# nmdp-bioinformatics/py-graph-imputation

Measured on AMD Instinct MI355X. Metric: imputed subjects/sec (whole node), 5-locus CAU graph, higher is better.
Workload: dtype f64; 1 GPU; BASELINE configs[1]: CAU 5-locus graph, 10k synthetic fully-typed subjects; 10000 subjects per step and GPU, seed=rank; graph_nodes=35411, populations=1

## Files before the change

include/grim_hip.h:

```cpp
#ifndef GRIM_HIP_H
#define GRIM_HIP_H

#include <stddef.h>
#include <stdint.h>

#ifdef __cplusplus
extern "C" {
#endif

#define GRIM_MAXL 5
#define GRIM_ABITS 12
#define GRIM_KEY_GRAPH_ORDER 60
#define GRIM_MAXPH 16
#define GRIM_MAXPOP 64
#define GRIM_TOPCAP 128
#define GRIM_MAXLADDER 64
#define GRIM_MAXROWS 8

typedef struct grim_ctx grim_ctx;
typedef struct grim_graph grim_graph;
typedef struct grim_batch grim_batch;

grim_ctx *grim_create(int device_id);
void grim_destroy(grim_ctx *ctx);
// ... 194 lines not shown

typedef struct {
  uint64_t lines, subjects, chunks, reruns;
  uint64_t unsupported;
  double wall_s;
  double tokenize_cpu_s, format_cpu_s, write_cpu_s;
  double device_s;
  double kernel_ms[7];
  uint64_t counters[4];
  uint64_t text_bytes[7];
  uint64_t bytes_h2d, bytes_d2h;
} grim_stream_stats;

grim_stream *grim_stream_open(grim_ctx *ctx, const grim_graph *g, const grim_dict *dict, const grim_params *prm,
                              const grim_prior_spec *priors, const char *const *pop_names, uint32_t n_pops,
                              const grim_stream_opts *opts);
int grim_stream_write(grim_stream *s, const char *text, uint64_t len);
int grim_stream_write_borrowed(grim_stream *s, const char *text, uint64_t len);
int grim_stream_write_text(grim_stream *s, const char *text, uint64_t len);
int grim_stream_write_file(grim_stream *s, const char *path);
int grim_stream_segment(grim_stream *s, uint64_t next_line_offset);
uint32_t grim_stream_n_segments(const grim_stream *s);
int grim_stream_segment_end(const grim_stream *s, uint32_t k, uint64_t out[7]);
int grim_stream_segment_wait(grim_stream *s, uint32_t k, uint64_t sizes[7]);
int grim_stream_segment_place(grim_stream *s, uint32_t k, const uint64_t base[6]);
int64_t grim_chunk_offsets(const char *path, uint32_t chunk_lines, uint64_t **out);
void grim_free(void *p);
uint32_t grim_default_threads(void);
int grim_stream_finish(grim_stream *s);
const char *grim_stream_error(const grim_stream *s);
const char *grim_stream_text(grim_stream *s, int which, uint64_t *len);
int grim_stream_get_stats(const grim_stream *s, grim_stream_stats *out);
int grim_stream_devtok_lines(const grim_stream *s, uint64_t *offered, uint64_t *handed_back);
uint32_t grim_tokname_hash(const char *name, uint32_t len);
uint64_t grim_stream_n_unsupported(const grim_stream *s);
int grim_stream_unsupported(const grim_stream *s, uint64_t k, uint64_t *line, uint32_t *reason, const char **id, uint32_t *id_len);
typedef struct {
  uint64_t first_line;
  uint32_t n_lines;
  const uint8_t *kinds;
  const grim_subject_result *res;
  const grim_row *rows;
  void *chunk;
} grim_stream_records;
int grim_stream_next_records(grim_stream *s, grim_stream_records *out);
int grim_stream_release_records(grim_stream *s, grim_stream_records *rec);
void grim_stream_free(grim_stream *s);

typedef struct grim_em grim_em;
typedef struct {
  uint64_t key;
  double w;
  uint32_t batch;
  uint32_t subject, row;
  uint16_t pop, side;
} grim_em_spill_rec;
grim_em *grim_em_create(grim_ctx *ctx, const uint32_t n_alleles[GRIM_MAXL], uint32_t n_pops, uint64_t first_capacity);
int grim_em_accumulate(grim_em *em, grim_batch *b);
int grim_em_accumulate_records(grim_em *em, const grim_subject_result *res, uint32_t n_subjects, const grim_row *rows,
                               uint64_t n_rows);
uint64_t grim_em_entries(const grim_em *em);
int grim_em_export(grim_em *em, uint64_t *keys, uint32_t *pops, double *counts);
uint64_t grim_em_spill_count(const grim_em *em);
int grim_em_spill(grim_em *em, uint64_t first, uint64_t n, grim_em_spill_rec *out);
int grim_em_stats(const grim_em *em, uint64_t out[4]);
uint64_t grim_em_last_unsupported(const grim_em *em);
// ... 83 lines not shown
```

py-graph-imputation_amd/csrc/grim_engine.hip:

```cpp
#include <hip/hip_runtime.h>
#include <hip/hip_ext.h>
#include <stdio.h>
#include <stdlib.h>
#include <string.h>
#include <algorithm>
#include <atomic>
#include <mutex>
#include <string>
#include <vector>

#include "grim_plan_a.h"
#include "grim_plan_b.h"
#include "grim_small.h"
#include "grim_medium.h"
#include "grim_mid.h"
#include "grim_tables.h"
#include "grim_tokdev.h"
#include "grim_em.h"
#include "grim_refresh.h"
#include "grim_marginal.h"
#include "grim_match.h"
#include "grim_search.h"
#include "grim_engine_internal.h"
#include "grim_host_internal.h"
#include "grim_sdma.h"

__global__ __launch_bounds__(GRIM_WG, GRIM_WG_PER_CU) void grim_plan_a_kernel(DevArgs A) {
  __shared__ WgShared sh;
  __shared__ WaveTop wt[GRIM_NWAVE];
  const int tid = threadIdx.x;
  const int P = A.g.P;
  Slot S = make_slot(A, blockIdx.x);
  const uint32_t n_bail = A.bail_list ? A.queue[GRIM_Q_BAIL] : 0, n_bail_heavy = A.bail_list ? A.queue[GRIM_Q_BAIL_HEAVY] : 0;
  const uint32_t n_mid = A.mid_list ? A.queue[GRIM_Q_MID] : 0;
  if (tid < GRIM_NWAVE * 4) ((unsigned long long *)sh.wctr)[tid] = 0;
  wg_arena(sh, wt);
  __syncthreads();
  for (;;) {
    if (tid == 0) sh.bc[3] = atomicAdd(A.queue + GRIM_Q_GENERAL, 1u);
    __syncthreads();
    const uint32_t w = sh.bc[3];
    if (A.mid_list ? w >= n_mid : w >= A.n_work + n_bail + n_bail_heavy) break;
    uint32_t si;
    if (A.mid_list)
      si = A.mid_list[w];
    else if (w < n_bail_heavy)
      si = A.bail_list[A.n_medium - 1u - w];
    else if (w - n_bail_heavy < A.n_work)
      si = A.order[w - n_bail_heavy];
    else
// ... 1189 lines not shown
  if (g2 == 0) g2 = 1;
  static int bucket_per_cu = 0;
  if (bucket_per_cu == 0) {
    int nb = 0;
    if (hipOccupancyMaxActiveBlocksPerMultiprocessor(&nb, grim_tables_bucket_kernel, 64, 0) != hipSuccess || nb <= 0) {
      (void)hipGetLastError();
      nb = 8;
    }
    bucket_per_cu = nb > 32 ? 32 : nb;
  }
  const uint32_t g3 = (uint32_t)c->n_cu * (uint32_t)bucket_per_cu;
  uint32_t g4 = (uint32_t)c->n_cu * (160u * 1024u / (uint32_t)sizeof(SplitWave)), g5 = (uint32_t)c->n_cu * 16u;
  if (g4 > cand) g4 = cand;
  if (g5 > cand) g5 = cand;
  if (g4 == 0) g4 = 1;
  if (g5 == 0) g5 = 1;
  (void)hipMemsetAsync(c->wctr, 0, 4 * GRIM_WCTR_WORDS, c->stream);
  launch_span(b, PH_TABLES, true, false, grim_tables_wave_kernel, dim3(g1), dim3(64), A);
  launch(b, PH_NONE, grim_tables_split_wave_kernel, dim3(g4), dim3(64), A);
  launch(b, PH_NONE, grim_tables_split_kernel, dim3(g2), dim3(GRIM_WG), A);
  launch(b, PH_NONE, grim_tables_bucket_kernel, dim3(g3), dim3(64), A);
  launch(b, PH_NONE, grim_tables_merge_wave_kernel, dim3(g5), dim3(64), A);
  launch_span(b, PH_TABLES, false, true, grim_tables_merge_kernel, dim3(g2), dim3(GRIM_WG), A);
}

static void enqueue_half_wave(grim_batch *b, bool timed, const DevArgs &Ak, const SmallRec *recs, const uint32_t *order, uint32_t n, uint32_t stage) {
  const uint32_t per_block = GRIM_WG / 32;
  launch(b, timed ? PH_HALF_WAVE : PH_NONE, grim_plan_a_small_kernel, dim3((n + per_block - 1) / per_block), dim3(GRIM_WG), Ak, recs, n, stage,
         b->small_stride);
  launch(b, timed ? PH_COMPACT : PH_NONE, grim_small_compact_kernel, dim3((n + 63) / 64), dim3(64), b->a, order, order ? nullptr : recs, n, stage,
         b->small_stride);
}

static int enqueue_stage1(grim_batch *b) {
  grim_ctx *c = b->ctx;
  DevArgs &A = b->a;
  const uint32_t stage0 = (uint32_t)b->row_limit - (b->n_small + b->n_dev_lines) * b->small_stride;
  if (b->n_small) enqueue_half_wave(b, b->n_dev_lines == 0, A, b->d_small, b->d_os, b->n_small, stage0);
  if (b->n_dev_lines) {
    DevTok T;
    T.text = b->d_text;
    T.lines = b->d_lines;
    T.lo = b->dev_lo;
    T.hi = b->dev_hi;
    T.dict = b->dict->d;
    T.dsmall = b->d_dsmall;
    T.subj = const_cast<grim_subject *>(A.subj);
    T.tok = const_cast<uint16_t *>(A.tok);
    T.tok_base = (uint32_t)(b->plan.tok_cap ? b->plan.tok_cap : 1);
    T.graph_loci = A.g.n_loci;
    const dim3 tgrid((b->n_dev_lines + (GRIM_WG / 64) * TOK_LINES_PER_WAVE - 1) / ((GRIM_WG / 64) * TOK_LINES_PER_WAVE));
    launch(b, PH_TOKENIZER, grim_tokenize_kernel, tgrid, dim3(GRIM_WG), A, T);
    DevArgs A2 = A;
    A2.small_ctr = A.small_ctr + 2 * b->n_host_small_waves;
    enqueue_half_wave(b, true, A2, b->d_dsmall, nullptr, b->n_dev_lines, stage0 + b->n_small * b->small_stride);
  }
  if (b->n_medium) {
    static const int waves_per_cu = env_int("GRIM_MEDIUM_WAVES", GRIM_MEDIUM_WAVES_PER_CU);
    uint32_t grid = (uint32_t)c->n_cu * (uint32_t)(waves_per_cu > 0 ? waves_per_cu : GRIM_MEDIUM_WAVES_PER_CU);
    if (grid > b->n_medium) grid = b->n_medium;
    launch(b, PH_ONE_WAVE, grim_plan_a_medium_kernel, dim3(grid), dim3(64), A, b->d_om, b->n_medium, A.bail_list);
  }
  if (A.mid_list && b->n_general + b->n_medium) {
    const uint32_t want = b->n_general + b->n_medium;
    uint32_t grid = (uint32_t)c->n_cu * GRIM_MID_WG_PER_CU;
    if (grid > want) grid = want;
    launch(b, PH_MID, grim_plan_a_mid_kernel, dim3(grid), dim3(GRIM_WG), A);
  }
  if (b->n_general + b->n_medium) {
    uint32_t want = b->n_general + b->n_medium;
    launch(b, PH_GENERAL, grim_plan_a_kernel, dim3(b->n_slots < want ? b->n_slots : want), dim3(GRIM_WG), A);
  }
  launch(b, PH_NONE, grim_finish_kernel, dim3(1), dim3(GRIM_WG), A.counters, b->hstate, 0u, 0);
  return hipGetLastError() == hipSuccess ? 0 : -1;
}

extern "C" int grim_batch_set_timing(grim_batch *b, int on) {
  if (!b) return -1;
  b->timing = on != 0;
  memset(b->acc_ms, 0, sizeof(b->acc_ms));
  b->n_timed = 0;
  return 0;
}

int engine_batch_upload_done(grim_batch *b) {
  if (!b || !b->up_pending) return 1;
  use_device(b->ctx->device);
  if (hipEventQuery(b->ev_up) == hipSuccess) return 1;
  (void)hipGetLastError();
  return 0;
}

int engine_batch_enqueue(grim_batch *b) {
  if (!b) return -1;
  grim_ctx *c = b->ctx;
  use_device(c->device);
  if (((uint64_t)b->n_small + b->n_dev_lines) * b->small_stride > b->row_limit) {
    b->rows_used = 0;
    set_err(c, "grim_batch_run: output row pool smaller than the half-wave kernel's fixed region");
    return -2;
  }
  memset(b->ms, 0, sizeof(b->ms));
  b->launched = 0;
  std::lock_guard<std::mutex> lk(c->run_mu);
  if (bind_scratch(b) != 0) return -1;
  if (b->up_pending) {
    b->up_pending = false;
    if (hipEventQuery(b->ev_up) != hipSuccess) {
      (void)hipGetLastError();
      HIPCHK(hipStreamWaitEvent(c->stream, b->ev_up, 0), c, -1);
    }
  }
  if (b->timing) {
    if (enqueue_stage1(b) != 0) {
      set_err(c, "grim_batch_run: kernel launch failed");
      return -1;
    }
  } else {
    if (b->graph_state == 0) {
      b->graph_state = -1;
      static const int use_graph = env_int("GRIM_GRAPH", 0);
      if (use_graph && hipStreamBeginCapture(c->stream, hipStreamCaptureModeThreadLocal) == hipSuccess) {
        int rc = enqueue_stage1(b);
        hipGraph_t gr = nullptr;
        hipError_t e = hipStreamEndCapture(c->stream, &gr);
        if (rc == 0 && e == hipSuccess && gr && hipGraphInstantiate(&b->gexec, gr, nullptr, nullptr, 0) == hipSuccess)
          b->graph_state = 1;
        if (gr) hipGraphDestroy(gr);
        (void)hipGetLastError();
      }
// ... 1463 lines not shown
```

py-graph-imputation_amd/csrc/grim_engine_internal.h:

```cpp
#pragma once
#include <stdint.h>

#include "../../include/grim_hip.h"
#include "grim_layout.h"
#include "grim_tok.h"

struct EnginePlan {
  uint32_t n_subj;
  uint64_t tok_cap;
  uint64_t text_cap;
};

struct EngineHost {
  grim_subject *subj;
  uint16_t *tok;
  SmallRec *small;
  uint32_t *order_s, *order_m, *order_g;
  grim_subject_result *res;
  grim_row *rows;
  LineRec *lines;
  uint8_t *text;
};

struct EngineLoad {
  uint32_t n_subj;
  uint32_t n_small, n_medium, n_general;
  uint64_t tok_used;
  uint32_t n_priors;
  const double *priors;
  uint32_t dev_lo, dev_hi;
  uint64_t text_bytes;
};

grim_batch *engine_batch_create(grim_ctx *ctx, const grim_graph *g, const grim_params *p, uint64_t row_limit, const EnginePlan *plan);
int engine_batch_plan(grim_batch *b, const EnginePlan *plan);
const EngineHost *engine_batch_host(grim_batch *b);
uint32_t engine_small_stride(const grim_params *p);
uint64_t engine_rows_per_subject(const grim_params *p, uint32_t n_pops);
int engine_batch_load(grim_batch *b, const EngineLoad *ld);
int engine_batch_fetch(grim_batch *b, uint32_t res_lo, uint32_t res_hi, grim_row *rows_dst);
uint64_t engine_bytes_moved(const grim_batch *b, int dir);
void engine_set_error(grim_ctx *ctx, const char *msg);
void engine_batch_recycle(grim_batch *b);
int engine_batch_fetch_issue(grim_batch *b);
int engine_batch_fetch_wait(grim_batch *b);
int engine_batch_upload_done(grim_batch *b);
int engine_batch_enqueue(grim_batch *b);
int engine_batch_wait(grim_batch *b);
struct DictSnap;
typedef struct grim_devdict grim_devdict;
grim_devdict *engine_devdict_create(grim_ctx *ctx, const DictSnap *snap);
void engine_devdict_free(grim_devdict *d);
void engine_batch_set_dict(grim_batch *b, const grim_devdict *d);
uint32_t engine_batch_irregular(const grim_batch *b);
uint32_t engine_graph_order_bad(const grim_graph *g);
uint64_t engine_batch_pool_want(const grim_batch *b);
void engine_batch_hint_pool(grim_batch *b, uint64_t records);
int engine_batch_grow_pool(grim_batch *b, uint64_t max_records);
int engine_batch_grow_rows(grim_batch *b, uint64_t max_rows);
uint64_t engine_batch_row_limit(const grim_batch *b);
void engine_batch_hint_rows(grim_batch *b, uint64_t rows);
```

py-graph-imputation_amd/csrc/grim_small.h:

```cpp
#pragma once
#include "grim_pair.h"


__device__ __forceinline__ double half_shfl_d(double v, int src_in_half) {
  return __shfl(v, (threadIdx.x & 32) | src_in_half);
}
__device__ __forceinline__ uint32_t half_shfl_u(uint32_t v, int src_in_half) {
  return __shfl(v, (threadIdx.x & 32) | src_in_half);
}

template <int CTRL>
__device__ __forceinline__ double dpp_d(double v) {
  const long long b = __double_as_longlong(v);
  const int lo = __builtin_amdgcn_update_dpp(0, (int)(uint32_t)b, CTRL, 0xF, 0xF, false);
  const int hi = __builtin_amdgcn_update_dpp(0, (int)(uint32_t)((unsigned long long)b >> 32), CTRL, 0xF, 0xF, false);
  return __longlong_as_double((long long)(((unsigned long long)(uint32_t)hi << 32) | (uint32_t)lo));
}
__device__ __forceinline__ double row16_max(double v) {
  double o;
  o = dpp_d<0x121>(v); v = o > v ? o : v;
  o = dpp_d<0x122>(v); v = o > v ? o : v;
  o = dpp_d<0x124>(v); v = o > v ? o : v;
  o = dpp_d<0x128>(v); v = o > v ? o : v;
  return v;
}

__global__ __launch_bounds__(GRIM_WG) void grim_plan_a_small_kernel(DevArgs A, const SmallRec *recs, uint32_t n,
                                                                   uint32_t row_base, uint32_t row_stride) {
  const DevGraph &g = A.g;
  const int hl = threadIdx.x & 31;
  const uint32_t w = blockIdx.x * (GRIM_WG / 32) + (threadIdx.x >> 5);
  bool live = w < n;
  const int n_ladder = A.prm.n_ladder;
  double lad[8];
#pragma unroll
  for (int i = 0; i < 8; ++i) lad[i] = A.prm.ladder[i];
  bool hit = false;
  uint64_t mykey = 0;
  double f = 0.0;
  uint32_t same = 0, si = 0;
  double w_prior = 0.0;
  if (live) {
    const uint4 *rp = (const uint4 *)(recs + w);
    const uint4 r0 = rp[0], r1 = rp[1];
    const uint32_t words[8] = {r0.x, r0.y, r0.z, r0.w, r1.x, r1.y, r1.z, r1.w};
    same = (words[6] >> 8) & 0xFFu;
    si = words[7];
    live = si != GRIM_NONE;
    w_prior = live ? A.priors[(uint64_t)(words[6] >> 16)] : 0.0;
#pragma unroll
    for (int l = 0; l < GRIM_MAXL; ++l) {
      const uint32_t tw = words[l];
      const uint32_t t = ((hl >> l) & 1) ? (tw >> 16) : (tw & 0xFFFFu);
      const uint32_t slot = (l < 4 ? (words[5] >> (8 * l)) : words[6]) & 0xFFu;
      mykey |= (uint64_t)(t + 1u) << (GRIM_ABITS * slot);
    }
    uint32_t h = fht_hash(mykey) & g.fht_mask;
    for (; live;) {
      const FullEnt e = g.fht[h];
      if (e.key == mykey) { hit = true; f = e.f0; break; }
      if (e.key == 0) break;
      h = (h + 1) & g.fht_mask;
    }
  }
  const bool hit2 = half_shfl_u(hit ? 1u : 0u, hl ^ 31) != 0;
  const double f2 = half_shfl_d(f, hl ^ 31);
  const uint64_t key2 = ((uint64_t)half_shfl_u((uint32_t)(mykey >> 32), hl ^ 31) << 32) | half_shfl_u((uint32_t)mykey, hl ^ 31);
  const uint32_t het4 = 15u & ~same;
  bool kept = hl < 16 && ((uint32_t)hl & ~het4 & 15u) == 0 && (!((same >> 4) & 1u) || ((uint32_t)hl ^ het4) >= (uint32_t)hl);
  const bool pair_ok = live && kept && f > 0.0 && f2 > 0.0;
  const bool same_hap = mykey == key2;
  PairRef pr;
  pr.p1 = f; pr.p2 = f2; pr.m2 = f2;
  pr.e1 = same_hap ? 0u : 1u; pr.e2 = 0u;
  const bool hi_half = (threadIdx.x & 32) != 0;
  double eps = 0.0;
// ... 16 lines not shown
    for (int idx = 0; idx < 8; ++idx)
      if (idx < n_ladder && (need_lo || need_hi)) step(lad[idx]);
    for (int idx = 8; idx < n_ladder && (need_lo || need_hi); ++idx) step(A.prm.ladder[idx]);
    eps = hi_half ? eps_hi : eps_lo;
    found = hi_half ? got_hi : got_lo;
  }
  double prob = acc ? pair_prob(pr, w_prior) : 0.0;
  double mx = row16_max(prob);
  if (found && eps > 0.0) {
    eps = mx / 100000.0;
    acc = pair_ok && pair_accept(eps, pr, w_prior);
    prob = acc ? pair_prob(pr, w_prior) : 0.0;
    mx = row16_max(prob);
  }
  const uint64_t bal = __ballot(acc);
  const uint32_t accmask = (uint32_t)(hi_half ? (bal >> 32) : bal) & 0xFFFFu;
  const uint32_t nU = __popc(accmask);
  double total = 0.0;
  bool first = true;
  uint32_t rank = 0;
  for (uint32_t um = ((uint32_t)bal | (uint32_t)(bal >> 32)) & 0xFFFFu; um; um &= um - 1) {
    const int i = __builtin_ctz(um);
    const double p_lo = lane_get(prob, i), p_hi = lane_get(prob, 32 + i);
    const double pi = hi_half ? p_hi : p_lo;
    if ((accmask >> i) & 1u) {
      total = first ? pi : total + pi;
      first = false;
      if (pi > prob || (pi == prob && i < hl)) ++rank;
    }
  }
  {
    const uint64_t need = __ballot(live && kept), needp = __ballot(live && kept && hit),
                   needq = __ballot(live && kept && hit2);
    if ((threadIdx.x & 63) == 0) {
      const uint32_t gw = blockIdx.x * (GRIM_WG / 64) + (threadIdx.x >> 6);
      *(uint2 *)(A.small_ctr + 2 * gw) = make_uint2(2u * (uint32_t)__popcll(need), (uint32_t)(__popcll(needp) + __popcll(needq)));
    }
  }
  if (!live) return;
  const uint32_t off = row_base + w * row_stride;
  const bool ok = nU > 0;
  const int first_lane = ok ? (__ffs(accmask) - 1) : 0;
  const uint32_t n_pm = (ok && A.prm.out_haps) ? (nU < A.prm.n_results ? nU : A.prm.n_results) : 0;
  const uint64_t ka = ((uint64_t)half_shfl_u((uint32_t)(mykey >> 32), first_lane) << 32) | half_shfl_u((uint32_t)mykey, first_lane);
  const uint64_t kb = ((uint64_t)half_shfl_u((uint32_t)(key2 >> 32), first_lane) << 32) | half_shfl_u((uint32_t)key2, first_lane);
  {
    const int f = hl - 16;
    const bool phase = hl < 16;
    const bool wr = ok && (phase ? (acc && rank < n_pm) : f == 0);
    if (wr) {
      grim_row r;
      r.a = phase ? mykey : ka;
      r.b = phase ? key2 : kb;
      r.prob = phase ? prob : total;
      r.popa = 0;
      r.popb = 0;
      A.rows[off + (phase ? GRIM_SMALL_ROWS_FIXED + rank : (uint32_t)f)] = r;
    }
  }
  if (hl >= 19 && hl < 26) {
    const int j = hl - 19;
    const uint8_t status = ok ? GRIM_ST_OK : (A.prm.planb ? GRIM_ST_UNSUPPORTED : GRIM_ST_MISS);
    const uint32_t head = (uint32_t)status | ((uint32_t)'a' << 8) | ((!ok && A.prm.planb) ? (2u << 16) : 0u);
    const uint32_t n_um = (ok && A.prm.out_muug && A.prm.n_results) ? 1u : 0u;
    const uint32_t n_up = (ok && A.prm.out_muug && A.prm.n_pop_results) ? 1u : 0u;
    const uint32_t n_pp = (ok && A.prm.out_haps && A.prm.n_pop_results) ? 1u : 0u;
    const uint64_t mxb = ok ? (uint64_t)__double_as_longlong(mx) : 0ull;
    uint32_t lo, hi;
    switch (j) {
      case 0: lo = head; hi = ok ? nU : 0u; break;
      case 1: lo = ok ? 1u : 0u; hi = ok ? off + 0 : 0u; break;
      case 2: lo = ok ? off + 0 : 0u; hi = ok ? off + GRIM_SMALL_ROWS_FIXED : 0u; break;
      case 3: lo = ok ? off + 0 : 0u; hi = n_um; break;
      case 4: lo = n_up; hi = n_pm; break;
      case 5: lo = n_pp; hi = 0u; break;
      default: lo = (uint32_t)mxb; hi = (uint32_t)(mxb >> 32); break;
    }
    ((uint2 *)(A.res + si))[j] = make_uint2(lo, hi);
  }
  if (!ok && hl == 0 && A.prm.planb) push_next(A, si, false);
}
```

py-graph-imputation_amd/csrc/grim_stream.cpp:

```cpp
#include <errno.h>
#include <execinfo.h>
#include <fcntl.h>
#include <signal.h>
#include <sched.h>
#include <hip/hip_runtime_api.h>
#include <stdint.h>
#include <stdio.h>
#include <stdlib.h>
#include <string.h>
#include <sys/stat.h>
#include <sys/types.h>
#include <unistd.h>
#if defined(__x86_64__)
#include <immintrin.h>
#endif

#include <algorithm>
#include <atomic>
#include <chrono>
#include <condition_variable>
#include <deque>
#include <memory>
#include <mutex>
#include <string>
// ... 1468 lines not shown
    for (auto &b : s->mem[which]) {
      s->joined[which].append(b.first, b.second);
      free(b.first);
    }
    s->mem[which].clear();
    s->joined_ok[which] = true;
  }
  if (len) *len = s->joined[which].size();
  return s->joined[which].data();
}

extern "C" int grim_stream_get_stats(const grim_stream *s, grim_stream_stats *out) {
  if (!s || !out) return -1;
  {
    std::lock_guard<std::mutex> lk(const_cast<grim_stream *>(s)->mu);
    *out = s->st;
  }
  out->tokenize_cpu_s = s->tok_ns.load() * 1e-9;
  out->format_cpu_s = s->fmt_ns.load() * 1e-9;
  out->write_cpu_s = s->wr_ns.load() * 1e-9;
  out->unsupported = s->unsupported.size();
  out->bytes_h2d = engine_bytes_moved(nullptr, 0);
  out->bytes_d2h = engine_bytes_moved(nullptr, 1);
  return 0;
}

extern "C" int grim_stream_devtok_lines(const grim_stream *s, uint64_t *offered, uint64_t *handed_back) {
  if (!s) return -1;
  if (offered) *offered = s->offered.load();
  if (handed_back) *handed_back = s->handed_back.load();
  return 0;
}

extern "C" uint64_t grim_stream_n_unsupported(const grim_stream *s) { return s ? s->unsupported.size() : 0; }

extern "C" int grim_stream_unsupported(const grim_stream *s, uint64_t k, uint64_t *line, uint32_t *reason, const char **id, uint32_t *id_len) {
  if (!s || k >= s->unsupported.size()) return -1;
  const auto &u = s->unsupported[k];
  if (line) *line = u.line;
  if (reason) *reason = u.reason;
  if (id) *id = u.id.data();
  if (id_len) *id_len = (uint32_t)u.id.size();
  return 0;
}

extern "C" int grim_stream_next_records(grim_stream *s, grim_stream_records *out) {
  if (!s || !out || !s->opt.want_records) return -1;
  std::unique_lock<std::mutex> lk(s->mu);
  for (;;) {
    if (s->failed) return -1;
    Chunk *c = s->by_index(s->next_record);
    if (c && c->state >= CH_COMMITTED && !c->records_out) {
      c->records_out = true;
      tl_note(c, 8);
      ++s->next_record;
      out->first_line = c->first_line;
      out->n_lines = c->n_lines;
      out->kinds = c->kinds.data();
      out->res = engine_batch_host(c->batch)->res;
      out->rows = c->rows;
      out->chunk = c;
      return 1;
    }
    if (s->input_closed && s->next_record >= s->next_index) return 0;
    const auto tw0 = Clock::now();
    s->cv_rec.wait_for(lk, std::chrono::milliseconds(50));
// ... 231 lines not shown
```

py-graph-imputation_amd/csrc/grim_tokdev.h:

```cpp
#pragma once
#include "grim_dev.h"
#include "grim_tok.h"

struct DevTok {
  const uint8_t *text;
  const LineRec *lines;
  uint32_t lo, hi;
  DevDict dict;
  SmallRec *dsmall;
  grim_subject *subj;
  uint16_t *tok;
  uint32_t tok_base;
  uint32_t graph_loci;
};
#define GRIM_REASON_HOST_TOKENIZER 7

#define TOK_LANES (2 * GRIM_MAXL)
#define TOK_LINES_PER_WAVE (64 / TOK_LANES)

__global__ __launch_bounds__(GRIM_WG) void grim_tokenize_kernel(DevArgs A, DevTok T) {
  const int lane = lane_id();
  const int a = lane % TOK_LANES, lw = lane / TOK_LANES;
  const uint32_t idx = (blockIdx.x * (GRIM_WG / 64) + wave_id()) * TOK_LINES_PER_WAVE + lw;
  const uint32_t line = T.lo + idx;
  const bool in_grid = lw < TOK_LINES_PER_WAVE && line < T.hi;
  LineRec lr;
  lr.gl_off = 0; lr.gl_len = 0; lr.prior_idx = 0;
  if (in_grid) lr = T.lines[line];
  const bool active = in_grid && lr.gl_len != 0;
  bool bad = active && lr.gl_len > GRIM_TOK_MAXGL;
  const uint32_t n = (active && !bad) ? lr.gl_len : 0;
  __shared__ uint4 lbuf[GRIM_WG / 64][TOK_LINES_PER_WAVE + 1][TOK_LANES];
  uint4 *mybuf = lbuf[wave_id()][lw < TOK_LINES_PER_WAVE ? lw : TOK_LINES_PER_WAVE];
  const uint32_t a0 = lr.gl_off & ~15u, skip = lr.gl_off - a0, tot = n ? skip + n : 0;
  uint4 q = make_uint4(0, 0, 0, 0);
  if (16u * (uint32_t)a < tot) q = ((const uint4 *)(T.text + a0))[a];
  mybuf[a] = q;
  uint32_t m_sep = 0, m_plus = 0;
  {
    const uint32_t wd[4] = {q.x, q.y, q.z, q.w};
#pragma unroll
    for (int bb = 0; bb < 16; ++bb) {
      const uint32_t pos = 16u * (uint32_t)a + (uint32_t)bb;
      const uint32_t c = (wd[bb >> 2] >> (8 * (bb & 3))) & 0xFFu;
      const bool in = pos >= skip && pos < tot;
      if (in && c == '+') m_plus |= 1u << bb;
      if (in && (c == '+' || c == '^')) m_sep |= 1u << bb;
      if (in && (c == '/' || c == 'g' || c == 'L')) bad = true;
    }
  }
  WAVE_SYNC();
  uint32_t nsep = 0, start = 0, end = n;
  {
    const int base0 = lw * TOK_LANES;
#pragma unroll
    for (int v = 0; v < TOK_LANES; ++v) {
      const int src = base0 + v < 64 ? base0 + v : 0;
      uint32_t mv = (uint32_t)__shfl((int)m_sep, src);
      const uint32_t pv = (uint32_t)__shfl((int)m_plus, src);
      const uint32_t c = (uint32_t)__popc(mv);
      if (a > 0 && nsep < (uint32_t)a && nsep + c >= (uint32_t)a) {
        uint32_t m2 = mv;
        for (uint32_t k = nsep; k + 1 < (uint32_t)a; ++k) m2 &= m2 - 1;
        start = 16u * (uint32_t)v + (uint32_t)__builtin_ctz(m2) + 1u - skip;
      }
      if (nsep <= (uint32_t)a && nsep + c > (uint32_t)a) {
// ... 61 lines not shown
    const int partner = lane ^ 1;
    const int pslot = __shfl(slot, partner);
    bool eq = __shfl((int)len, partner) == (int)len;
#pragma unroll
    for (int i = 0; i < 6; ++i) eq = eq && __shfl((int)w[i], partner) == (int)w[i];
    if (active && !bad && pslot != slot) bad = true;
    const int nxt = lane + 2;
    bool less = false, decided = false;
#pragma unroll
    for (int i = 0; i < 6; ++i) {
      const uint32_t o = (uint32_t)__shfl((int)w[i], nxt < 64 ? nxt : lane);
      if (!decided && o != w[i]) {
        less = w[i] < o;
        decided = true;
      }
    }
    if (active && !bad && a + 2 < TOK_LANES && !(decided && less)) bad = true;
#pragma unroll
    for (int k = 0; k < GRIM_MAXL; ++k) {
      const int src = base + 2 * k;
      const int sk = __shfl(slot, src < 64 ? src : 0);
      const int ek = __shfl(eq ? 1 : 0, src < 64 ? src : 0);
      if (sk >= 0) {
        used |= 1u << sk;
        slots5 |= (uint32_t)sk << (4 * k);
      }
      same |= (uint32_t)(ek & 1) << k;
    }
  }
  const uint64_t badm = __ballot(bad);
  const uint32_t line_bad = (uint32_t)(badm >> base) & ((1u << TOK_LANES) - 1u);
  const bool ok = active && line_bad == 0 && __popc(used) == GRIM_MAXL && T.graph_loci == GRIM_MAXL && T.dict.n_loci == GRIM_MAXL;
  if (!in_grid) return;
  SmallRec *rec = T.dsmall + idx;
  if (ok) {
    rec->tok[a] = (uint16_t)id;
    T.tok[(uint64_t)T.tok_base + (uint64_t)TOK_LANES * line + a] = (uint16_t)id;
    if ((a & 1) == 0) rec->slot[a >> 1] = (uint8_t)slot;
  }
  if (a == 0) {
    if (ok) {
      rec->same = (uint8_t)same;
      rec->prior_idx = lr.prior_idx;
      rec->si = line;
      grim_subject sj;
      sj.tok_off = T.tok_base + TOK_LANES * line;
      sj.prior_idx = lr.prior_idx;
      sj.n_loci = GRIM_MAXL;
      sj.flags = 0;
#pragma unroll
      for (int k = 0; k < GRIM_MAXL; ++k) {
        sj.slot[k] = (uint8_t)((slots5 >> (4 * k)) & 0xFu);
        sj.cnt[k][0] = sj.cnt[k][1] = 1;
        sj.wid[k][0] = sj.wid[k][1] = 1;
      }
      sj.pad[0] = (uint8_t)same;
      sj.pad[1] = sj.pad[2] = 0;
      sj.reserved[0] = sj.reserved[1] = 0;
      T.subj[line] = sj;
    } else {
      rec->si = GRIM_NONE;
      if (active) {
        uint32_t *r = (uint32_t *)(A.res + line);
        r[0] = (uint32_t)GRIM_ST_UNSUPPORTED | ((uint32_t)'a' << 8) | ((uint32_t)GRIM_REASON_HOST_TOKENIZER << 16);
        atomicAdd(A.queue + GRIM_Q_IRREGULAR, 1u);
      }
    }
  }
}
```

py-graph-imputation_amd/grim/_native.py:

```python

import ctypes as C
import os

import numpy as np

MAXL = 5
ABITS = 12
MAXPH = 16
MAXPOP = 64
TOPCAP = 128
MAXLADDER = 64
MAXROWS = 8

ST_OK, ST_MISS, ST_UNSUPPORTED, ST_NOPHASE = 0, 1, 2, 3
T_UMUG, T_UMUG_POPS, T_PMUG, T_PMUG_POPS = 0, 1, 2, 3
(MS_TOTAL, MS_PLAN_A, MS_PLAN_B, MS_HALF_WAVE, MS_GENERAL, MS_ONE_WAVE, MS_TABLES, MS_COMPACT, MS_TOKENIZER,
 MS_MID) = range(10)
MS_MEAN = 0x10

_HERE = os.path.dirname(os.path.abspath(__file__))
LIB_PATH = os.environ.get("GRIM_LIB") or os.path.join(os.path.dirname(_HERE), "libgrim_hip.so")


class GraphDesc(C.Structure):
# ... 705 lines not shown
        return hits, n_hits

    def flags(self):
        n_p, n_d = self.patients(), self.donors()
        pf, df = np.zeros(n_p, dtype=np.uint8), np.zeros(n_d, dtype=np.uint8)
        self._check(_search_lib().grim_search_flags(self.h, _ptr(pf) if n_p else None, _ptr(df) if n_d else None), "grim_search_flags",
                    code=False)
        return pf, df

    def stats(self):
        out = (C.c_uint64 * 8)()
        _search_lib().grim_search_stats(self.h, out)
        return {k: int(v) for k, v in zip(SEARCH_STATS, out)}

    def kernel_ms(self):
        return float(_search_lib().grim_search_kernel_ms(self.h))

    def select_ms(self):
        return float(_search_lib().grim_search_select_ms(self.h))


K_DEVICE, K_PROBLEM_ID, K_PROBLEM_RAW, K_MISS_NO_DEVICE, K_UNSUPPORTED, K_UNSUPPORTED_GL = 0, 1, 2, 3, 4, 5

EXPORTS += [
    "grim_dict_create", "grim_dict_free", "grim_dict_set_locus", "grim_dict_intern", "grim_dict_find", "grim_dict_name",
    "grim_dict_count", "grim_tokenize", "grim_parsed_free", "grim_parsed_lines", "grim_parsed_subjects",
    "grim_parsed_subject_array", "grim_parsed_tokens", "grim_parsed_kinds", "grim_parsed_dev_index",
    "grim_parsed_n_races", "grim_parsed_race", "grim_parsed_id", "grim_parsed_set_kind", "grim_parsed_set_flags", "grim_format", "grim_text_get", "grim_text_free",
    "grim_format_double", "grim_hostgraph_load_csv", "grim_hostgraph_desc", "grim_hostgraph_free", "grim_graphgen_csv", "grim_hostgraph_from_hpf",
    "grim_parsed_allele", "grim_prior_matrix", "grim_stream_open", "grim_stream_write", "grim_stream_write_borrowed", "grim_stream_write_file", "grim_stream_finish",
    "grim_stream_error", "grim_stream_text", "grim_stream_get_stats", "grim_stream_n_unsupported", "grim_stream_unsupported",
    "grim_stream_next_records", "grim_stream_release_records", "grim_stream_free", "grim_stream_write_text",
    "grim_stream_segment", "grim_stream_n_segments", "grim_stream_segment_end", "grim_stream_segment_wait", "grim_stream_segment_place", "grim_default_threads", "grim_chunk_offsets", "grim_free",
    "grim_stream_devtok_lines", "grim_tokname_hash",
]


class PriorSpec(C.Structure):
    _fields_ = [("alpha", C.c_double), ("eta", C.c_double), ("beta", C.c_double), ("gamma", C.c_double), ("delta", C.c_double),
                ("unk_mr", C.c_uint8), ("count_by_prob", C.POINTER(C.c_double))]


class StreamOpts(C.Structure):
    _fields_ = [("chunk_lines", C.c_uint32), ("depth", C.c_uint32), ("n_threads", C.c_int32), ("line_offset", C.c_uint64),
                ("rows_per_chunk", C.c_uint64), ("want_text", C.c_uint8), ("want_log", C.c_uint8), ("want_records", C.c_uint8),
                ("timing", C.c_uint8), ("rows_exact", C.c_uint8), ("placed", C.c_uint8), ("out_path", C.c_char_p * 6), ("mask_ids", C.c_char_p), ("mask_fixed", C.c_void_p),
                ("n_masks", C.c_uint32)]


class StreamStats(C.Structure):
    _fields_ = [("lines", C.c_uint64), ("subjects", C.c_uint64), ("chunks", C.c_uint64), ("reruns", C.c_uint64),
                ("unsupported", C.c_uint64), ("wall_s", C.c_double), ("tokenize_cpu_s", C.c_double), ("format_cpu_s", C.c_double),
                ("write_cpu_s", C.c_double), ("device_s", C.c_double), ("kernel_ms", C.c_double * 7), ("counters", C.c_uint64 * 4),
                ("text_bytes", C.c_uint64 * 7), ("bytes_h2d", C.c_uint64), ("bytes_d2h", C.c_uint64)]


class StreamRecords(C.Structure):
    _fields_ = [("first_line", C.c_uint64), ("n_lines", C.c_uint32), ("kinds", C.c_void_p), ("res", C.c_void_p),
                ("rows", C.c_void_p), ("chunk", C.c_void_p)]


_host_ready = False


def host_lib():
    global _host_ready
    L = lib()
# ... 70 lines not shown
    L.grim_stream_write_file.argtypes = [C.c_void_p, C.c_char_p]
    L.grim_stream_finish.restype = C.c_int
    L.grim_stream_finish.argtypes = [C.c_void_p]
    L.grim_stream_error.restype = C.c_char_p
    L.grim_stream_error.argtypes = [C.c_void_p]
    L.grim_stream_text.restype = C.c_void_p
    L.grim_stream_text.argtypes = [C.c_void_p, C.c_int, C.POINTER(C.c_uint64)]
    L.grim_stream_get_stats.restype = C.c_int
    L.grim_stream_get_stats.argtypes = [C.c_void_p, C.POINTER(StreamStats)]
    L.grim_stream_n_unsupported.restype = C.c_uint64
    L.grim_stream_n_unsupported.argtypes = [C.c_void_p]
    L.grim_stream_unsupported.restype = C.c_int
    L.grim_stream_unsupported.argtypes = [C.c_void_p, C.c_uint64, C.POINTER(C.c_uint64), C.POINTER(C.c_uint32), C.POINTER(C.c_void_p),
                                          C.POINTER(C.c_uint32)]
    L.grim_stream_next_records.restype = C.c_int
    L.grim_stream_next_records.argtypes = [C.c_void_p, C.POINTER(StreamRecords)]
    L.grim_stream_release_records.restype = C.c_int
    L.grim_stream_release_records.argtypes = [C.c_void_p, C.POINTER(StreamRecords)]
    L.grim_stream_free.argtypes = [C.c_void_p]
    L.grim_stream_write_text.restype = C.c_int
    L.grim_stream_write_text.argtypes = [C.c_void_p, C.c_char_p, C.c_uint64]
    L.grim_stream_segment.restype = C.c_int
    L.grim_stream_segment.argtypes = [C.c_void_p, C.c_uint64]
    L.grim_stream_n_segments.restype = C.c_uint32
    L.grim_stream_n_segments.argtypes = [C.c_void_p]
    L.grim_stream_segment_end.restype = C.c_int
    L.grim_stream_segment_end.argtypes = [C.c_void_p, C.c_uint32, C.POINTER(C.c_uint64)]
    L.grim_stream_segment_wait.restype = C.c_int
    L.grim_stream_segment_wait.argtypes = [C.c_void_p, C.c_uint32, C.POINTER(C.c_uint64)]
    L.grim_stream_segment_place.restype = C.c_int
    L.grim_stream_segment_place.argtypes = [C.c_void_p, C.c_uint32, C.POINTER(C.c_uint64)]
    L.grim_stream_devtok_lines.restype = C.c_int
    L.grim_stream_devtok_lines.argtypes = [C.c_void_p, C.POINTER(C.c_uint64), C.POINTER(C.c_uint64)]
    L.grim_tokname_hash.restype = C.c_uint32
    L.grim_tokname_hash.argtypes = [C.c_char_p, C.c_uint32]
    L.grim_default_threads.restype = C.c_uint32
    L.grim_chunk_offsets.restype = C.c_int64
    L.grim_chunk_offsets.argtypes = [C.c_char_p, C.c_uint32, C.POINTER(C.POINTER(C.c_uint64))]
    L.grim_free.argtypes = [C.c_void_p]
    _host_ready = True
    return L


def tokname_hash(name):
    b = name.encode() if isinstance(name, str) else bytes(name)
    return int(host_lib().grim_tokname_hash(b, len(b)))


def host_threads():
    n = int(os.environ.get("GRIM_HOST_THREADS", "0"))
    if n <= 0:
        n = min(16, os.cpu_count() or 1)
    return n


class AlleleDict:

    def __init__(self, slot_locus):
        L = host_lib()
        self.n = len(slot_locus)
        self.h = L.grim_dict_create(self.n)
        if not self.h:
            raise NativeError("grim_dict_create failed")
        for s, name in enumerate(slot_locus):
            L.grim_dict_set_locus(self.h, s, name.encode())
        self._cache = [dict() for _ in slot_locus]
# ... 284 lines not shown
        return out

    def segment_wait(self, k):
        v = (C.c_uint64 * 7)()
        self._check(host_lib().grim_stream_segment_wait(self.h, int(k), v))
        return [int(x) for x in v]

    def segment_place(self, k, base):
        v = (C.c_uint64 * 6)(*[int(x) for x in base])
        self._check(host_lib().grim_stream_segment_place(self.h, int(k), v))

    def write_file(self, path):
        self._check(host_lib().grim_stream_write_file(self.h, os.fsencode(path)))

    def finish(self):
        self._check(host_lib().grim_stream_finish(self.h))

    def text(self, which, as_bytes=False):
        n = C.c_uint64(0)
        ptr = host_lib().grim_stream_text(self.h, which, C.byref(n))
        data = C.string_at(ptr, n.value) if n.value else b""
        return data if as_bytes else data.decode()

    def stats(self):
        st = StreamStats()
        host_lib().grim_stream_get_stats(self.h, C.byref(st))
        return st

    def devtok_lines(self):
        a, b = C.c_uint64(0), C.c_uint64(0)
        self._check(host_lib().grim_stream_devtok_lines(self.h, C.byref(a), C.byref(b)))
        return int(a.value), int(b.value)

    def unsupported(self):
        L = host_lib()
        out = []
        for k in range(int(L.grim_stream_n_unsupported(self.h))):
            line, reason, ptr, n = C.c_uint64(0), C.c_uint32(0), C.c_void_p(0), C.c_uint32(0)
            L.grim_stream_unsupported(self.h, k, C.byref(line), C.byref(reason), C.byref(ptr), C.byref(n))
            out.append((int(line.value), C.string_at(ptr.value, n.value).decode() if n.value else "", int(reason.value)))
        return out

    def next_records(self):
        rec = StreamRecords()
        rc = host_lib().grim_stream_next_records(self.h, C.byref(rec))
        self._check(rc)
        if rc == 0:
            return None
        n = int(rec.n_lines)
        kinds = np.frombuffer((C.c_char * n).from_address(rec.kinds), dtype=np.uint8, count=n)
        res = np.frombuffer((C.c_char * (n * RESULT_DT.itemsize)).from_address(rec.res), dtype=RESULT_DT, count=n)
        return int(rec.first_line), kinds, res, rec.rows, rec

    def release(self, rec):
        host_lib().grim_stream_release_records(self.h, C.byref(rec))

    def close(self):
        if self.h:
            host_lib().grim_stream_free(self.h)
            self.h = None
        self._lent = []

    def __del__(self):
        try:
            self.close()
        except Exception:
# ... 2 lines not shown
```

Before: 173.3 million subjects/s.

## Fuse device tokenizer and half-wave small kernel into one chunk kernel

When a batch contains only device-tokenized lines, one chunk kernel now tokenizes a group of lines into LDS, runs the half-wave subject imputation on them, and stages the output rows in shared memory. A single scan-and-atomicAdd per block then packs the rows compactly into the row pool instead of reserving a fixed per-subject region. This removes one kernel launch and the global round-trip of SmallRec records, and stops wasting row-pool space on the fixed staging stride. In exchange the block needs a large LDS footprint, which can limit occupancy, and it adds an overflow path plus a wide/narrow variant chosen by grid size. It is skipped when per-phase timing is enabled.

```diff
diff --git a/include/grim_hip.h b/include/grim_hip.h
--- a/include/grim_hip.h
+++ b/include/grim_hip.h
@@ -250,6 +250,7 @@
 const char *grim_stream_text(grim_stream *s, int which, uint64_t *len);
 int grim_stream_get_stats(const grim_stream *s, grim_stream_stats *out);
 int grim_stream_devtok_lines(const grim_stream *s, uint64_t *offered, uint64_t *handed_back);
+int grim_stream_chunk_launches(const grim_stream *s, uint64_t *launches);
 uint32_t grim_tokname_hash(const char *name, uint32_t len);
 uint64_t grim_stream_n_unsupported(const grim_stream *s);
 int grim_stream_unsupported(const grim_stream *s, uint64_t k, uint64_t *line, uint32_t *reason, const char **id, uint32_t *id_len);
diff --git a/py-graph-imputation_amd/csrc/grim_chunk.h b/py-graph-imputation_amd/csrc/grim_chunk.h
--- /dev/null
+++ b/py-graph-imputation_amd/csrc/grim_chunk.h
@@ -0,0 +1,91 @@
+#pragma once
+#include "grim_small.h"
+#include "grim_tokdev.h"
+
+#define CHUNK_LINES (GRIM_NWAVE * TOK_LINES_PER_WAVE)
+#define CHUNK_PAIRS (CHUNK_LINES / 2)
+#define CHUNK_ROWS_MAX (GRIM_SMALL_ROWS_FIXED + 16)
+#define CHUNK_WAVES_WIDE 12
+#define CHUNK_WAVES_NARROW GRIM_NWAVE
+#define CHUNK_WIDE_WG_PER_CU 2
+static_assert(CHUNK_LINES % 2 == 0 && CHUNK_PAIRS % CHUNK_WAVES_WIDE == 0 && CHUNK_PAIRS % CHUNK_WAVES_NARROW == 0, "whole rounds of subject pairs");
+
+struct ChunkHead {
+  uint32_t si;
+  uint32_t nU, n_pm, ok;
+  double mx;
+};
+
+struct ChunkShared {
+  TokWaveBuf lbuf[GRIM_NWAVE];
+  SmallRec recs[CHUNK_LINES];
+  grim_row rows[CHUNK_LINES][CHUNK_ROWS_MAX];
+  ChunkHead head[CHUNK_LINES];
+  uint32_t off[CHUNK_LINES], cnt[CHUNK_LINES];
+  uint32_t overflow;
+};
+
+struct ChunkSink {
+  ChunkShared &sh;
+  uint32_t s;
+  __device__ __forceinline__ void row(uint32_t k, const grim_row &r) { sh.rows[s][k] = r; }
+  __device__ __forceinline__ void header(uint32_t si, int j, bool ok, uint32_t nU, uint32_t n_pm, double mx) {
+    if (j == 0) sh.head[s] = ChunkHead{si, nU, n_pm, ok ? 1u : 0u, mx};
+  }
+};
+
+template <int WAVES>
+__global__ __launch_bounds__(64 * WAVES) void grim_chunk_kernel(DevArgs A, DevTok T, uint32_t n_cells) {
+  __shared__ ChunkShared sh;
+  const int tid = threadIdx.x;
+  const uint32_t idx0 = blockIdx.x * CHUNK_LINES;
+  if (tid < CHUNK_LINES) {
+    sh.head[tid].si = GRIM_NONE;
+    if (T.lo + idx0 + tid >= T.hi) sh.recs[tid].si = GRIM_NONE;
+  }
+  if (wave_id() < GRIM_NWAVE)
+    tokenize_group(A, T, idx0 + wave_id() * TOK_LINES_PER_WAVE, sh.lbuf[wave_id()], sh.recs + wave_id() * TOK_LINES_PER_WAVE);
+  __syncthreads();
+  for (uint32_t p = wave_id(); p < CHUNK_PAIRS; p += WAVES) {
+    const uint32_t s = 2 * p + ((tid >> 5) & 1);
+    const uint32_t cell = blockIdx.x * CHUNK_PAIRS + p;
+    ChunkSink sink{sh, s};
+    half_wave_subject(A, sh.recs + s, T.lo + idx0 + s < T.hi, cell < n_cells ? A.small_ctr + 2 * cell : nullptr, sink);
+  }
+  __syncthreads();
+  if (wave_id() == 0) {
+    const int lane = lane_id();
+    uint32_t cnt = 0;
+    if (lane < CHUNK_LINES) {
+      const ChunkHead h = sh.head[lane];
+      const bool any = (A.prm.out_muug && (A.prm.n_results || A.prm.n_pop_results)) || h.n_pm || (A.prm.out_haps && A.prm.n_pop_results);
+      if (h.si != GRIM_NONE && h.ok && any) cnt = GRIM_SMALL_ROWS_FIXED + h.n_pm;
+    }
+    const uint32_t incl = wave_incl_scan(cnt);
+    const uint32_t total = __shfl(incl, 63);
+    uint32_t base = 0;
+    if (lane == 0 && total) base = atomicAdd(A.row_head, total);
+    base = __shfl(base, 0);
+    const bool full = total && (uint64_t)base + total > A.row_cap;
+    if (lane == 0) {
+      sh.overflow = full ? 1u : 0u;
+      if (full) run_overflow(A);
+    }
+    if (lane < CHUNK_LINES) {
+      sh.off[lane] = base + incl - cnt;
+      sh.cnt[lane] = cnt;
+    }
+  }
+  __syncthreads();
+  if (sh.overflow) return;
+  for (uint32_t i = tid; i < CHUNK_LINES * 2 * CHUNK_ROWS_MAX; i += 64 * WAVES) {
+    const uint32_t s = i / (2 * CHUNK_ROWS_MAX), k = i % (2 * CHUNK_ROWS_MAX);
+    if (k < 2 * sh.cnt[s]) ((uint4 *)(A.rows + sh.off[s]))[k] = ((const uint4 *)sh.rows[s])[k];
+  }
+  for (uint32_t i = tid; i < CHUNK_LINES * 7; i += 64 * WAVES) {
+    const uint32_t s = i / 7;
+    const int j = (int)(i % 7);
+    const ChunkHead h = sh.head[s];
+    if (h.si != GRIM_NONE) ((uint2 *)(A.res + h.si))[j] = small_header_piece(A.prm, j, h.ok != 0, h.nU, h.n_pm, h.mx, sh.off[s]);
+  }
+}
diff --git a/py-graph-imputation_amd/csrc/grim_engine.hip b/py-graph-imputation_amd/csrc/grim_engine.hip
--- a/py-graph-imputation_amd/csrc/grim_engine.hip
+++ b/py-graph-imputation_amd/csrc/grim_engine.hip
@@ -16,6 +16,7 @@
 #include "grim_mid.h"
 #include "grim_tables.h"
 #include "grim_tokdev.h"
+#include "grim_chunk.h"
 #include "grim_em.h"
 #include "grim_refresh.h"
 #include "grim_marginal.h"
@@ -1271,10 +1272,20 @@
          b->small_stride);
 }
 
+static std::atomic<uint64_t> g_chunk_launches{0};
+uint64_t engine_chunk_launches() { return g_chunk_launches.load(); }
+
+static bool chunk_kernel_wanted(const grim_batch *b) {
+  return b->n_dev_lines > 0 && b->n_small == 0 && b->n_medium == 0 && b->n_general == 0 && !b->timing && env_int("GRIM_CHUNK_KERNEL", 1) != 0;
+}
+
 static int enqueue_stage1(grim_batch *b) {
   grim_ctx *c = b->ctx;
   DevArgs &A = b->a;
-  const uint32_t stage0 = (uint32_t)b->row_limit - (b->n_small + b->n_dev_lines) * b->small_stride;
+  const bool chunk = chunk_kernel_wanted(b);
+  const uint64_t staged = chunk ? 0 : ((uint64_t)b->n_small + b->n_dev_lines) * b->small_stride;
+  A.row_cap = (uint32_t)(b->row_limit - (staged <= b->row_limit ? staged : 0));
+  const uint32_t stage0 = A.row_cap;
   if (b->n_small) enqueue_half_wave(b, b->n_dev_lines == 0, A, b->d_small, b->d_os, b->n_small, stage0);
   if (b->n_dev_lines) {
     DevTok T;
@@ -1288,11 +1299,20 @@
     T.tok = const_cast<uint16_t *>(A.tok);
     T.tok_base = (uint32_t)(b->plan.tok_cap ? b->plan.tok_cap : 1);
     T.graph_loci = A.g.n_loci;
-    const dim3 tgrid((b->n_dev_lines + (GRIM_WG / 64) * TOK_LINES_PER_WAVE - 1) / ((GRIM_WG / 64) * TOK_LINES_PER_WAVE));
-    launch(b, PH_TOKENIZER, grim_tokenize_kernel, tgrid, dim3(GRIM_WG), A, T);
-    DevArgs A2 = A;
-    A2.small_ctr = A.small_ctr + 2 * b->n_host_small_waves;
-    enqueue_half_wave(b, true, A2, b->d_dsmall, nullptr, b->n_dev_lines, stage0 + b->n_small * b->small_stride);
+    if (chunk) {
+      const uint32_t grid = (b->n_dev_lines + CHUNK_LINES - 1) / CHUNK_LINES;
+      if (grid <= CHUNK_WIDE_WG_PER_CU * (uint32_t)c->n_cu)
+        launch(b, PH_NONE, grim_chunk_kernel<CHUNK_WAVES_WIDE>, dim3(grid), dim3(64 * CHUNK_WAVES_WIDE), A, T, b->n_small_waves);
+      else
+        launch(b, PH_NONE, grim_chunk_kernel<CHUNK_WAVES_NARROW>, dim3(grid), dim3(64 * CHUNK_WAVES_NARROW), A, T, b->n_small_waves);
+      g_chunk_launches++;
+    } else {
+      const dim3 tgrid((b->n_dev_lines + (GRIM_WG / 64) * TOK_LINES_PER_WAVE - 1) / ((GRIM_WG / 64) * TOK_LINES_PER_WAVE));
+      launch(b, PH_TOKENIZER, grim_tokenize_kernel, tgrid, dim3(GRIM_WG), A, T);
+      DevArgs A2 = A;
+      A2.small_ctr = A.small_ctr + 2 * b->n_host_small_waves;
+      enqueue_half_wave(b, true, A2, b->d_dsmall, nullptr, b->n_dev_lines, stage0 + b->n_small * b->small_stride);
+    }
   }
   if (b->n_medium) {
     static const int waves_per_cu = env_int("GRIM_MEDIUM_WAVES", GRIM_MEDIUM_WAVES_PER_CU);
@@ -1334,7 +1354,7 @@
   if (!b) return -1;
   grim_ctx *c = b->ctx;
   use_device(c->device);
-  if (((uint64_t)b->n_small + b->n_dev_lines) * b->small_stride > b->row_limit) {
+  if (!chunk_kernel_wanted(b) && ((uint64_t)b->n_small + b->n_dev_lines) * b->small_stride > b->row_limit) {
     b->rows_used = 0;
     set_err(c, "grim_batch_run: output row pool smaller than the half-wave kernel's fixed region");
     return -2;
diff --git a/py-graph-imputation_amd/csrc/grim_engine_internal.h b/py-graph-imputation_amd/csrc/grim_engine_internal.h
--- a/py-graph-imputation_amd/csrc/grim_engine_internal.h
+++ b/py-graph-imputation_amd/csrc/grim_engine_internal.h
@@ -46,6 +46,7 @@
 int engine_batch_fetch_wait(grim_batch *b);
 int engine_batch_upload_done(grim_batch *b);
 int engine_batch_enqueue(grim_batch *b);
+uint64_t engine_chunk_launches();
 int engine_batch_wait(grim_batch *b);
 struct DictSnap;
 typedef struct grim_devdict grim_devdict;
diff --git a/py-graph-imputation_amd/csrc/grim_small.h b/py-graph-imputation_amd/csrc/grim_small.h
--- a/py-graph-imputation_amd/csrc/grim_small.h
+++ b/py-graph-imputation_amd/csrc/grim_small.h
@@ -25,12 +25,30 @@
   return v;
 }
 
-__global__ __launch_bounds__(GRIM_WG) void grim_plan_a_small_kernel(DevArgs A, const SmallRec *recs, uint32_t n,
-                                                                   uint32_t row_base, uint32_t row_stride) {
+__device__ __forceinline__ uint2 small_header_piece(const grim_params &prm, int j, bool ok, uint32_t nU, uint32_t n_pm, double mx, uint32_t off) {
+  const uint8_t status = ok ? GRIM_ST_OK : (prm.planb ? GRIM_ST_UNSUPPORTED : GRIM_ST_MISS);
+  const uint32_t head = (uint32_t)status | ((uint32_t)'a' << 8) | ((!ok && prm.planb) ? (2u << 16) : 0u);
+  const uint32_t n_um = (ok && prm.out_muug && prm.n_results) ? 1u : 0u;
+  const uint32_t n_up = (ok && prm.out_muug && prm.n_pop_results) ? 1u : 0u;
+  const uint32_t n_pp = (ok && prm.out_haps && prm.n_pop_results) ? 1u : 0u;
+  const uint64_t mxb = ok ? (uint64_t)__double_as_longlong(mx) : 0ull;
+  uint32_t lo, hi;
+  switch (j) {
+    case 0: lo = head; hi = ok ? nU : 0u; break;
+    case 1: lo = ok ? 1u : 0u; hi = ok ? off + 0 : 0u; break;
+    case 2: lo = ok ? off + 0 : 0u; hi = ok ? off + GRIM_SMALL_ROWS_FIXED : 0u; break;
+    case 3: lo = ok ? off + 0 : 0u; hi = n_um; break;
+    case 4: lo = n_up; hi = n_pm; break;
+    case 5: lo = n_pp; hi = 0u; break;
+    default: lo = (uint32_t)mxb; hi = (uint32_t)(mxb >> 32); break;
+  }
+  return make_uint2(lo, hi);
+}
+
+template <class Sink>
+__device__ __forceinline__ void half_wave_subject(const DevArgs &A, const SmallRec *rec, bool live, uint32_t *ctr_cell, Sink &sink) {
   const DevGraph &g = A.g;
   const int hl = threadIdx.x & 31;
-  const uint32_t w = blockIdx.x * (GRIM_WG / 32) + (threadIdx.x >> 5);
-  bool live = w < n;
   const int n_ladder = A.prm.n_ladder;
   double lad[8];
 #pragma unroll
@@ -41,7 +59,7 @@
   uint32_t same = 0, si = 0;
   double w_prior = 0.0;
   if (live) {
-    const uint4 *rp = (const uint4 *)(recs + w);
+    const uint4 *rp = (const uint4 *)rec;
     const uint4 r0 = rp[0], r1 = rp[1];
     const uint32_t words[8] = {r0.x, r0.y, r0.z, r0.w, r1.x, r1.y, r1.z, r1.w};
     same = (words[6] >> 8) & 0xFFu;
@@ -124,13 +142,10 @@
   {
     const uint64_t need = __ballot(live && kept), needp = __ballot(live && kept && hit),
                    needq = __ballot(live && kept && hit2);
-    if ((threadIdx.x & 63) == 0) {
-      const uint32_t gw = blockIdx.x * (GRIM_WG / 64) + (threadIdx.x >> 6);
-      *(uint2 *)(A.small_ctr + 2 * gw) = make_uint2(2u * (uint32_t)__popcll(need), (uint32_t)(__popcll(needp) + __popcll(needq)));
-    }
+    if ((threadIdx.x & 63) == 0 && ctr_cell)
+      *(uint2 *)ctr_cell = make_uint2(2u * (uint32_t)__popcll(need), (uint32_t)(__popcll(needp) + __popcll(needq)));
   }
   if (!live) return;
-  const uint32_t off = row_base + w * row_stride;
   const bool ok = nU > 0;
   const int first_lane = ok ? (__ffs(accmask) - 1) : 0;
   const uint32_t n_pm = (ok && A.prm.out_haps) ? (nU < A.prm.n_results ? nU : A.prm.n_results) : 0;
@@ -147,28 +162,25 @@
       r.prob = phase ? prob : total;
       r.popa = 0;
       r.popb = 0;
-      A.rows[off + (phase ? GRIM_SMALL_ROWS_FIXED + rank : (uint32_t)f)] = r;
+      sink.row(phase ? GRIM_SMALL_ROWS_FIXED + rank : (uint32_t)f, r);
     }
   }
-  if (hl >= 19 && hl < 26) {
-    const int j = hl - 19;
-    const uint8_t status = ok ? GRIM_ST_OK : (A.prm.planb ? GRIM_ST_UNSUPPORTED : GRIM_ST_MISS);
-    const uint32_t head = (uint32_t)status | ((uint32_t)'a' << 8) | ((!ok && A.prm.planb) ? (2u << 16) : 0u);
-    const uint32_t n_um = (ok && A.prm.out_muug && A.prm.n_results) ? 1u : 0u;
-    const uint32_t n_up = (ok && A.prm.out_muug && A.prm.n_pop_results) ? 1u : 0u;
-    const uint32_t n_pp = (ok && A.prm.out_haps && A.prm.n_pop_results) ? 1u : 0u;
-    const uint64_t mxb = ok ? (uint64_t)__double_as_longlong(mx) : 0ull;
-    uint32_t lo, hi;
-    switch (j) {
-      case 0: lo = head; hi = ok ? nU : 0u; break;
-      case 1: lo = ok ? 1u : 0u; hi = ok ? off + 0 : 0u; break;
-      case 2: lo = ok ? off + 0 : 0u; hi = ok ? off + GRIM_SMALL_ROWS_FIXED : 0u; break;
-      case 3: lo = ok ? off + 0 : 0u; hi = n_um; break;
-      case 4: lo = n_up; hi = n_pm; break;
-      case 5: lo = n_pp; hi = 0u; break;
-      default: lo = (uint32_t)mxb; hi = (uint32_t)(mxb >> 32); break;
-    }
-    ((uint2 *)(A.res + si))[j] = make_uint2(lo, hi);
-  }
+  if (hl >= 19 && hl < 26) sink.header(si, hl - 19, ok, nU, n_pm, mx);
   if (!ok && hl == 0 && A.prm.planb) push_next(A, si, false);
 }
+
+struct StagedSink {
+  const DevArgs &A;
+  uint32_t off;
+  __device__ __forceinline__ void row(uint32_t k, const grim_row &r) { A.rows[off + k] = r; }
+  __device__ __forceinline__ void header(uint32_t si, int j, bool ok, uint32_t nU, uint32_t n_pm, double mx) {
+    ((uint2 *)(A.res + si))[j] = small_header_piece(A.prm, j, ok, nU, n_pm, mx, off);
+  }
+};
+
+__global__ __launch_bounds__(GRIM_WG) void grim_plan_a_small_kernel(DevArgs A, const SmallRec *recs, uint32_t n,
+                                                                   uint32_t row_base, uint32_t row_stride) {
+  const uint32_t w = blockIdx.x * (GRIM_WG / 32) + (threadIdx.x >> 5);
+  StagedSink sink{A, row_base + w * row_stride};
+  half_wave_subject(A, recs + w, w < n, A.small_ctr + 2 * (blockIdx.x * (GRIM_WG / 64) + (threadIdx.x >> 6)), sink);
+}
diff --git a/py-graph-imputation_amd/csrc/grim_stream.cpp b/py-graph-imputation_amd/csrc/grim_stream.cpp
--- a/py-graph-imputation_amd/csrc/grim_stream.cpp
+++ b/py-graph-imputation_amd/csrc/grim_stream.cpp
@@ -1524,6 +1524,12 @@
   return 0;
 }
 
+extern "C" int grim_stream_chunk_launches(const grim_stream *s, uint64_t *launches) {
+  if (!s) return -1;
+  if (launches) *launches = engine_chunk_launches();
+  return 0;
+}
+
 extern "C" uint64_t grim_stream_n_unsupported(const grim_stream *s) { return s ? s->unsupported.size() : 0; }
 
 extern "C" int grim_stream_unsupported(const grim_stream *s, uint64_t k, uint64_t *line, uint32_t *reason, const char **id, uint32_t *id_len) {
diff --git a/py-graph-imputation_amd/csrc/grim_tokdev.h b/py-graph-imputation_amd/csrc/grim_tokdev.h
--- a/py-graph-imputation_amd/csrc/grim_tokdev.h
+++ b/py-graph-imputation_amd/csrc/grim_tokdev.h
@@ -18,11 +18,12 @@
 #define TOK_LANES (2 * GRIM_MAXL)
 #define TOK_LINES_PER_WAVE (64 / TOK_LANES)
 
-__global__ __launch_bounds__(GRIM_WG) void grim_tokenize_kernel(DevArgs A, DevTok T) {
+typedef uint4 TokWaveBuf[TOK_LINES_PER_WAVE + 1][TOK_LANES];
+
+__device__ __forceinline__ void tokenize_group(const DevArgs &A, const DevTok &T, uint32_t idx0, TokWaveBuf &wbuf, SmallRec *recs) {
   const int lane = lane_id();
   const int a = lane % TOK_LANES, lw = lane / TOK_LANES;
-  const uint32_t idx = (blockIdx.x * (GRIM_WG / 64) + wave_id()) * TOK_LINES_PER_WAVE + lw;
-  const uint32_t line = T.lo + idx;
+  const uint32_t line = T.lo + idx0 + lw;
   const bool in_grid = lw < TOK_LINES_PER_WAVE && line < T.hi;
   LineRec lr;
   lr.gl_off = 0; lr.gl_len = 0; lr.prior_idx = 0;
@@ -30,8 +31,7 @@
   const bool active = in_grid && lr.gl_len != 0;
   bool bad = active && lr.gl_len > GRIM_TOK_MAXGL;
   const uint32_t n = (active && !bad) ? lr.gl_len : 0;
-  __shared__ uint4 lbuf[GRIM_WG / 64][TOK_LINES_PER_WAVE + 1][TOK_LANES];
-  uint4 *mybuf = lbuf[wave_id()][lw < TOK_LINES_PER_WAVE ? lw : TOK_LINES_PER_WAVE];
+  uint4 *mybuf = wbuf[lw < TOK_LINES_PER_WAVE ? lw : TOK_LINES_PER_WAVE];
   const uint32_t a0 = lr.gl_off & ~15u, skip = lr.gl_off - a0, tot = n ? skip + n : 0;
   uint4 q = make_uint4(0, 0, 0, 0);
   if (16u * (uint32_t)a < tot) q = ((const uint4 *)(T.text + a0))[a];
@@ -159,7 +159,7 @@
   const uint32_t line_bad = (uint32_t)(badm >> base) & ((1u << TOK_LANES) - 1u);
   const bool ok = active && line_bad == 0 && __popc(used) == GRIM_MAXL && T.graph_loci == GRIM_MAXL && T.dict.n_loci == GRIM_MAXL;
   if (!in_grid) return;
-  SmallRec *rec = T.dsmall + idx;
+  SmallRec *rec = recs + lw;
   if (ok) {
     rec->tok[a] = (uint16_t)id;
     T.tok[(uint64_t)T.tok_base + (uint64_t)TOK_LANES * line + a] = (uint16_t)id;
@@ -195,3 +195,9 @@
     }
   }
 }
+
+__global__ __launch_bounds__(GRIM_WG) void grim_tokenize_kernel(DevArgs A, DevTok T) {
+  __shared__ TokWaveBuf lbuf[GRIM_WG / 64];
+  const uint32_t idx0 = (blockIdx.x * (GRIM_WG / 64) + wave_id()) * TOK_LINES_PER_WAVE;
+  tokenize_group(A, T, idx0, lbuf[wave_id()], T.dsmall + idx0);
+}
diff --git a/py-graph-imputation_amd/grim/_native.py b/py-graph-imputation_amd/grim/_native.py
--- a/py-graph-imputation_amd/grim/_native.py
+++ b/py-graph-imputation_amd/grim/_native.py
@@ -761,7 +761,7 @@
     "grim_stream_error", "grim_stream_text", "grim_stream_get_stats", "grim_stream_n_unsupported", "grim_stream_unsupported",
     "grim_stream_next_records", "grim_stream_release_records", "grim_stream_free", "grim_stream_write_text",
     "grim_stream_segment", "grim_stream_n_segments", "grim_stream_segment_end", "grim_stream_segment_wait", "grim_stream_segment_place", "grim_default_threads", "grim_chunk_offsets", "grim_free",
-    "grim_stream_devtok_lines", "grim_tokname_hash",
+    "grim_stream_devtok_lines", "grim_tokname_hash", "grim_stream_chunk_launches",
 ]
 
 
@@ -898,6 +898,8 @@
     L.grim_stream_segment_place.argtypes = [C.c_void_p, C.c_uint32, C.POINTER(C.c_uint64)]
     L.grim_stream_devtok_lines.restype = C.c_int
     L.grim_stream_devtok_lines.argtypes = [C.c_void_p, C.POINTER(C.c_uint64), C.POINTER(C.c_uint64)]
+    L.grim_stream_chunk_launches.restype = C.c_int
+    L.grim_stream_chunk_launches.argtypes = [C.c_void_p, C.POINTER(C.c_uint64)]
     L.grim_tokname_hash.restype = C.c_uint32
     L.grim_tokname_hash.argtypes = [C.c_char_p, C.c_uint32]
     L.grim_default_threads.restype = C.c_uint32
@@ -1248,6 +1250,11 @@
         self._check(host_lib().grim_stream_devtok_lines(self.h, C.byref(a), C.byref(b)))
         return int(a.value), int(b.value)
 
+    def chunk_launches(self):
+        n = C.c_uint64(0)
+        self._check(host_lib().grim_stream_chunk_launches(self.h, C.byref(n)))
+        return int(n.value)
+
     def unsupported(self):
         L = host_lib()
         out = []
```

Result: slower. 151.6 million subjects/s (-12.6%).
